# AlexIoannides/bodywork-mlops-demo

Hardware: NVIDIA H100
Metric: train rows/sec (N x 128 least-squares fit) (higher is better)
Workload: dtype bf16x2 (hi+lo) MMA operands, f32 accumulate, f64 fold+solve

## Files before the change

### bodywork-mlops-demo_b200/csrc/b2_api.cu

```cuda
#include <dlfcn.h>
#include <math.h>
#include <stdarg.h>
#include <stdlib.h>

#include <new>
#include <thread>
#include <vector>

#include "b2_internal.cuh"
#include "b2_xchg.cuh"

namespace b2 {

static thread_local char g_err[768] = "";

void set_error(const char* fmt, ...) {
  va_list ap;
  va_start(ap, fmt);
  vsnprintf(g_err, sizeof(g_err), fmt, ap);
  va_end(ap);
}

namespace {

// ... 55 lines not shown
  if (n < 0) { set_error("n_rows < 0"); return B2_E_ARG; }
  if (ldx < d) { set_error("ldx=%lld < d=%d", (long long)ldx, d); return B2_E_ARG; }
  if (mem_kind != B2_MEM_DEVICE && mem_kind != B2_MEM_HOST) { set_error("bad mem_kind %d", mem_kind); return B2_E_ARG; }
  return B2_OK;
}

constexpr int64_t kMaxRowsPerLaunch = (int64_t)1 << 30;

int gram_dispatch(b2_ctx* ctx, const void* X, int x_dtype, const float* y, int64_t n, int d, int64_t ldx,
                  const uint8_t* mask, int keep, bool* tc_last = nullptr, unsigned int* scatter_epoch = nullptr) {
  const int es = x_dtype == B2_F32 ? 4 : 2;
  for (int64_t r0 = 0; r0 < n; r0 += kMaxRowsPerLaunch) {
    const int64_t rows = n - r0 < kMaxRowsPerLaunch ? n - r0 : kMaxRowsPerLaunch;
    const char* Xb = static_cast<const char*>(X) + (size_t)r0 * ldx * es;
    const float* yb = y + r0;
    const uint8_t* mb = mask != nullptr ? mask + r0 : nullptr;
    const bool tc_ok = gram_tc_supported(Xb, x_dtype, yb, rows, d, ldx, mb);
    const bool nw_ok = gram_narrow_supported(Xb, x_dtype, yb, rows, d, ldx, mb);
    int mode = ctx->kernel_mode;
    if (mode == B2_KERNEL_TCGEN05 && !tc_ok) {
      set_error("tensor-core path needs d%%4==0 (fp32) / d%%8==0 (bf16), 16-byte aligned X/y/mask/row pitch, n>=32");
      return B2_E_UNSUPPORTED;
    }
    if (mode == B2_KERNEL_NARROW && !nw_ok) {
      set_error("narrow path needs d<=16, contiguous rows (ldx==d) and 16-byte aligned X/y/mask");
      return B2_E_UNSUPPORTED;
    }
    if (mode == B2_KERNEL_AUTO) {
      if (nw_ok && rows >= 4096) mode = B2_KERNEL_NARROW;
      else mode = (tc_ok && rows >= 2048) ? B2_KERNEL_TCGEN05 : B2_KERNEL_SIMT;
    }
    const int64_t main_rows = mode == B2_KERNEL_NARROW ? gram_narrow_main_rows(rows, d)
                            : mode == B2_KERNEL_TCGEN05 ? gram_tc_main_rows(rows, d, ldx, nullptr) : 0;
    if (main_rows > 0)
      if (int r = launch_gram_shift(ctx, Xb, x_dtype, yb, rows, d, ldx)) return r;
    if (main_rows < rows) {
      if (int r = launch_gram_simt(ctx, Xb + (size_t)main_rows * ldx * es, x_dtype, yb + main_rows, rows - main_rows, d,
                                   ldx, mb != nullptr ? mb + main_rows : nullptr, keep, ctx->s_zero_pending))
        return r;
      ctx->s_zero_pending = false;
    }
    const bool last = r0 + rows == n;
    if (main_rows > 0 && mode == B2_KERNEL_NARROW) {
      if (int r = launch_gram_narrow(ctx, Xb, x_dtype, yb, rows, d, mb, keep, ctx->s_zero_pending)) return r;
      ctx->s_zero_pending = false;
    } else if (main_rows > 0) {
      const unsigned int epoch =
          last && scatter_epoch != nullptr && ctx->n_ranks > 1 && ctx->p2p_ready ? ++ctx->xchg_epoch : 0u;
      if (int r = launch_gram_tc(ctx, Xb, x_dtype, yb, rows, d, ldx, mb, keep, ctx->s_zero_pending, epoch)) return r;
      ctx->s_zero_pending = false;
      if (scatter_epoch != nullptr) *scatter_epoch = epoch;
    }
    if (last && tc_last != nullptr) *tc_last = mode == B2_KERNEL_TCGEN05;
  }
  return B2_OK;
}

int ensure_staging(b2_ctx* ctx) {
  if (ctx->stage_x[0] != nullptr) return B2_OK;
  ctx->stage_rows = 1 << 18;
  ctx->stage_bytes_x = (size_t)ctx->stage_rows * kMaxD * 4;
  for (int b = 0; b < 2; ++b) {
    B2_CUDA(cudaMalloc(&ctx->stage_x[b], ctx->stage_bytes_x));
    B2_CUDA(cudaMalloc(reinterpret_cast<void**>(&ctx->stage_y[b]), (size_t)ctx->stage_rows * 4));
    B2_CUDA(cudaMalloc(reinterpret_cast<void**>(&ctx->stage_m[b]), (size_t)ctx->stage_rows));
    B2_CUDA(cudaEventCreateWithFlags(&ctx->ev_copied[b], cudaEventDisableTiming));
// ... 1596 lines not shown
```

### bodywork-mlops-demo_b200/csrc/b2_internal.cuh

```cuda
#pragma once
#include <cuda.h>
#include <cuda_bf16.h>
#include <cuda_runtime.h>
#include <stdint.h>
#include <stdio.h>
#include <string.h>

#include <type_traits>

#include "../../include/b2gram.h"

namespace b2 {

constexpr int kMaxD = B2_MAX_D;
constexpr int kMaxS = kMaxD + 2;
constexpr int kKernelEventPairs = 64;
constexpr int kMaxRanks = 8;
constexpr size_t kXchgSlotDoubles = (size_t)kMaxS * kMaxS;
constexpr size_t kXchgDataDoubles = 2 * kMaxRanks * kXchgSlotDoubles;
constexpr size_t kXchgBytes = kXchgDataDoubles * sizeof(double) + 256;

constexpr int kTcRows = 64;
constexpr int kTcM = 128;
constexpr int kTcEMax = 16;
// ... 76 lines not shown
  do {                                                                                     \
    cudaError_t e_ = (call);                                                               \
    if (e_ != cudaSuccess) {                                                               \
      b2::set_error("%s failed: %s (%s:%d)", #call, cudaGetErrorString(e_), __FILE__, __LINE__); \
      return B2_E_CUDA;                                                                    \
    }                                                                                      \
  } while (0)

}

struct b2_ctx {
  int device = 0;
  int sm_count = 0;
  size_t hbm_bytes = 0;
  char name[128] = {0};
  cudaStream_t stream = nullptr;
  cudaStream_t copy_stream = nullptr;
  cudaEvent_t ev_t0 = nullptr, ev_t1 = nullptr;
  cudaEvent_t ev_k[b2::kKernelEventPairs][2];
  int k_pairs = 0;
  int64_t launches = 0;

  int kernel_mode = B2_KERNEL_AUTO;
  int drain_rows = 8192;
  int precision = B2_PRECISION_SPLIT;

  int d = 0;
  double* S = nullptr;

  double* tc_part = nullptr;
  double* tc_red = nullptr;
  float* shift = nullptr;
  bool solve_attr_set = false;
  double* solve_host = nullptr;
  struct TmCache {
    const void* X = nullptr; const float* y = nullptr; const uint8_t* mask = nullptr;
    int64_t n = 0, ldx = 0; int d = 0, x_dtype = -1;
    int y_map_2d = 0, m_map_2d = 0;
    alignas(64) unsigned char tmX[128], tmY[128], tmM[128];
  } tm_cache;
  double* simt_part = nullptr;
  int simt_ctas = 0;
  double* score_part = nullptr;
  int score_ctas = 0;
  double* coef_dev = nullptr;
  double* grad_part = nullptr;
  double* refine = nullptr;
  double* loo = nullptr;
  double* loo_part = nullptr;
  double* cv_stage[2] = {nullptr, nullptr};
  int cv_stage_alphas = 0;
  double* enet = nullptr;
  size_t enet_doubles = 0;
  double* folds = nullptr;
  size_t folds_doubles = 0;
  int n_folds = 0;
  int folds_d = 0;
  unsigned long long* fold_range = nullptr;
  double* coef_host = nullptr;
  cudaEvent_t ev_coef[2] = {nullptr, nullptr};
  int coef_slot = 0;
  long long* synth_count = nullptr;
  double* solve_out = nullptr;
  void* stage_x[2] = {nullptr, nullptr};
  float* stage_y[2] = {nullptr, nullptr};
  uint8_t* stage_m[2] = {nullptr, nullptr};
// ... 101 lines not shown
```

### bodywork-mlops-demo_b200/csrc/b2_ptx.cuh

```cuda
#pragma once
#include <cuda_bf16.h>
#include <stdint.h>

namespace b2 {

__device__ __forceinline__ uint32_t smem_u32(const void* p) {
  return static_cast<uint32_t>(__cvta_generic_to_shared(p));
}
__device__ __forceinline__ void mbar_init(uint32_t bar, uint32_t count) {
  asm volatile("mbarrier.init.shared::cta.b64 [%0], %1;" ::"r"(bar), "r"(count));
}
__device__ __forceinline__ void mbar_arrive(uint32_t bar) {
  asm volatile("mbarrier.arrive.shared::cta.b64 _, [%0];" ::"r"(bar) : "memory");
}
__device__ __forceinline__ void mbar_expect_tx(uint32_t bar, uint32_t bytes) {
  asm volatile("mbarrier.arrive.expect_tx.shared::cta.b64 _, [%0], %1;" ::"r"(bar), "r"(bytes) : "memory");
}
__device__ __forceinline__ uint64_t globaltimer_ns() {
  uint64_t t;
  asm volatile("mov.u64 %0, %globaltimer;" : "=l"(t));
  return t;
}
__device__ __forceinline__ void mbar_wait(uint32_t bar, uint32_t parity, uint32_t hint_ns = 20000u) {
  uint32_t done = 0;
  uint64_t t0 = 0;
  while (true) {
    asm volatile(
        "{\n\t.reg .pred p;\n\t"
        "mbarrier.try_wait.parity.shared::cta.b64 p, [%1], %2, %3;\n\t"
        "selp.u32 %0, 1, 0, p;\n\t}"
        : "=r"(done)
        : "r"(bar), "r"(parity), "r"(hint_ns)
        : "memory");
    if (done) break;
    const uint64_t now = globaltimer_ns();
    if (t0 == 0) t0 = now;
    else if (now - t0 > 4000000000ull) __trap();
  }
}
__device__ __forceinline__ void fence_proxy_async_smem() {
  asm volatile("fence.proxy.async.shared::cta;" ::: "memory");
}

__device__ __forceinline__ float ld_shared_f32(uint32_t addr) {
  float v;
  asm volatile("ld.shared.f32 %0, [%1];" : "=f"(v) : "r"(addr));
  return v;
}
__device__ __forceinline__ uint32_t ld_shared_u8(uint32_t addr) {
  uint32_t v;
  asm volatile("ld.shared.u8 %0, [%1];" : "=r"(v) : "r"(addr));
  return v;
}
template <typename T>
__device__ __forceinline__ float raw_ld_shared(uint32_t addr);
template <>
__device__ __forceinline__ float raw_ld_shared<float>(uint32_t addr) { return ld_shared_f32(addr); }
template <>
__device__ __forceinline__ float raw_ld_shared<__nv_bfloat16>(uint32_t addr) {
  unsigned short h;
  asm volatile("ld.shared.u16 %0, [%1];" : "=h"(h) : "r"(addr));
  return __uint_as_float(((uint32_t)h) << 16);
}
template <typename T>
__device__ __forceinline__ float raw_ld_global(const T* p);
template <>
__device__ __forceinline__ float raw_ld_global<float>(const float* p) { return __ldg(p); }
template <>
__device__ __forceinline__ float raw_ld_global<__nv_bfloat16>(const __nv_bfloat16* p) {
  return __bfloat162float(*p);
}
// ... 113 lines not shown
```

### bodywork-mlops-demo_b200/csrc/gram_shift.cu

```cuda
#include <cuda_bf16.h>

#include "b2_internal.cuh"
#include "b2_ptx.cuh"

namespace b2 {
namespace {

constexpr int kShiftBlocks = 64;
constexpr int kShiftStride = kMaxD + 1;
constexpr int kShiftPartOff = kMaxD + 1;
constexpr int kShiftTicketOff = kShiftPartOff + kShiftBlocks * kShiftStride;

__host__ __device__ __forceinline__ int64_t shift_samples(int64_t n) { return n < 2048 ? n : 2048; }

__device__ __forceinline__ float shift_round(float c, bool round_bf16) {
  return round_bf16 ? __bfloat162float(__float2bfloat16_rn(c)) : c;
}
__device__ __noinline__ float shift_value(const float* sp, int j, bool round_bf16) {
  float acc = 0.f;
  int cnt = 0;
#pragma unroll 8
  for (int b = 0; b < kShiftBlocks; ++b) {
    const float p = sp[b * kShiftStride + j];
    if (p == p) { acc += p; ++cnt; }
  }
  return shift_round(cnt > 0 ? acc / (float)cnt : 0.f, round_bf16);
}

constexpr int kShiftCols = 160;
constexpr int kShiftGroups = 4;

template <typename T>
__global__ void __launch_bounds__(kShiftCols * kShiftGroups)
tc_shift_kernel(const T* __restrict__ X, const float* __restrict__ y, int64_t n, int d, int64_t ldx, float* shift) {
  __shared__ float sub[kShiftGroups][kShiftCols];
  __shared__ int subn[kShiftGroups][kShiftCols];
  __shared__ bool last_block;
  __shared__ float part_s[kShiftBlocks * kShiftStride];
  float* sp = shift + kShiftPartOff;
  const int j = threadIdx.x % kShiftCols, g = threadIdx.x / kShiftCols;
  const int64_t samples = shift_samples(n);
  const int64_t stride = n / samples;
  const int64_t per = (samples + kShiftBlocks - 1) / kShiftBlocks;
  const int64_t s0 = blockIdx.x * per;
  const int64_t s1 = (s0 + per < samples) ? s0 + per : samples;
  float acc = 0.f;
  int cnt = 0;
  if (j <= d) {
#pragma unroll 8
    for (int64_t s = s0 + g; s < s1; s += kShiftGroups) {
      const int64_t row = s * stride;
      const float v = (j < d) ? raw_ld_global<T>(X + row * ldx + j) : __ldg(y + row);
      const bool finite = fabsf(v) <= 3.0e38f;
      acc += finite ? v : 0.f;
      cnt += finite ? 1 : 0;
    }
  }
  sub[g][j] = acc;
  subn[g][j] = cnt;
  __syncthreads();
  if (g == 0 && j <= d) {
    const int c = subn[0][j] + subn[1][j] + subn[2][j] + subn[3][j];
    sp[blockIdx.x * kShiftStride + (j == d ? kMaxD : j)] =
        c > 0 ? (((sub[0][j] + sub[1][j]) + sub[2][j]) + sub[3][j]) / (float)c : __int_as_float(0x7fc00000);
    __threadfence();
  }
  __syncthreads();
  unsigned int* ticket = reinterpret_cast<unsigned int*>(shift + kShiftTicketOff);
  if (threadIdx.x == 0) last_block = atomicAdd(ticket, 1u) == gridDim.x - 1;
  __syncthreads();
  if (!last_block) return;
// ... 33 lines not shown
```

### bodywork-mlops-demo_b200/csrc/gram_tc.cu

```cuda
#include <cuda_bf16.h>
#include <stdlib.h>

#include "b2_internal.cuh"
#include "b2_ptx.cuh"
#include "b2_shift.cuh"
#include "b2_xchg.cuh"

namespace b2 {
namespace {

constexpr int kConsumerWGs = 2;
constexpr int kXformWarps = 8;
constexpr int kThreads = 128 * (kConsumerWGs + 2);
constexpr int kFirstXformWarp = 4 * kConsumerWGs;
constexpr int kTmaWarp = kFirstXformWarp;
constexpr int kEWarp = kFirstXformWarp + 1;
static_assert(kFirstXformWarp + kXformWarps == kThreads / 32, "warp roles");
constexpr int kProducers = kXformWarps;
constexpr int kConsumerWarps = 4 * kConsumerWGs;
constexpr int kKGroups = kTcRows / 8;
constexpr uint32_t kRawStageBytes = kTcRows * kMaxD * 4;
constexpr uint32_t kOpSBO = 128;
constexpr uint32_t kOpLBO = (16 + 2 + 16) * kOpSBO;
constexpr uint32_t kOpEOff = 16 * kOpSBO;
// ... 295 lines not shown
  uint8_t* smem = smem_raw + (sbase - smem_u32(smem_raw));
  const int warp = threadIdx.x >> 5;
  const int lane = threadIdx.x & 31;

  const uint32_t bar_raw_full = sbase + G::kOffBar;
  const uint32_t bar_raw_empty = bar_raw_full + 8 * kRawStages;
  const uint32_t bar_op_full = bar_raw_empty + 8 * kRawStages;
  const uint32_t bar_op_empty = bar_op_full + 8 * kOpStages;
  float* shift_s = reinterpret_cast<float*>(smem + G::kOffShift);

  const int64_t total_tiles = (n_rows + kTcRows - 1) / kTcRows;
  const int64_t tile_begin = (int64_t)blockIdx.x * total_tiles / gridDim.x;
  const int64_t tile_end = (int64_t)(blockIdx.x + 1) * total_tiles / gridDim.x;
  const int my_tiles = (int)(tile_end - tile_begin);

  if (threadIdx.x == 0) {
    for (int s = 0; s < kRawStages; ++s) {
      mbar_init(bar_raw_full + 8 * s, 1);
      mbar_init(bar_raw_empty + 8 * s, kProducers + (RAWB ? kConsumerWarps : 0));
    }
    for (int s = 0; s < kOpStages; ++s) {
      mbar_init(bar_op_full + 8 * s, kProducers);
      mbar_init(bar_op_empty + 8 * s, kConsumerWarps);
    }
    asm volatile("fence.mbarrier_init.release.cluster;" ::: "memory");
  }
  if (warp == kTmaWarp && lane == 0) {
    tma_prefetch_desc(&tmX);
    tma_prefetch_desc(&tmY);
    if (has_mask) tma_prefetch_desc(&tmM);
  }
  for (uint32_t o = threadIdx.x * 16; o < kOpStages * kOpStageBytes; o += kThreads * 16)
    *reinterpret_cast<uint4*>(smem + kOffOp + o) = make_uint4(0, 0, 0, 0);
  for (int j = threadIdx.x; j <= kMaxD; j += kThreads)
    shift_s[j] = j == kMaxD ? shift[kMaxD] : (j < pack * d_orig ? shift[j % d_orig] : 0.f);
  fence_proxy_async_smem();
  __syncthreads();

  if (warp < kConsumerWarps) {
    asm volatile("setmaxnreg.inc.sync.aligned.u32 %0;" ::"n"(G::kConsumerRegs));
    auto consume = [&](auto wg_c) {
      constexpr int WG = decltype(wg_c)::value;
      constexpr int kF1 = kTcM - 64 * WG;
      constexpr int kF2 = RAWB ? kF1 : kTcM;
      constexpr int kC1 = 64 * WG;
      constexpr int kR1 = (kF1 + EW) / 2, kR2 = (kF2 + EW) / 2;
      float acc1[kR1], acc2[kR2];
      double* my_part = part + (size_t)blockIdx.x * kTcAccElems;
      auto store = [&](auto n_regs, int dst_acc, int col0, bool add, auto val) {
        const int ln = (int)lane_id(), row0 = 64 * WG + 16 * (warp & 3) + (ln >> 2);
#pragma unroll
        for (int r = 0; r < decltype(n_regs)::value; ++r) {
          const int col = col0 + 8 * (r >> 2) + 2 * (ln & 3) + (r & 1), h = (r >> 1) & 1, i = row0 + 8 * h;
          const bool lower = dst_acc == 0 && col < kTcM && i > col;
          put_f64(my_part + tc_part_index(dst_acc, i, col, EW), val(r, col, h), add, !lower);
        }
      };
      auto drain = [&](const auto& acc, int dst_acc, int col0, bool add) {
        constexpr int kR = sizeof(acc) / sizeof(float);
        if constexpr (RAWB) {
          constexpr int kF = 2 * kR - EW;
          const double s1[2] = {(double)__shfl_sync(0xffffffffu, acc[kF / 2], lane & ~3),
                                (double)__shfl_sync(0xffffffffu, acc[kF / 2 + 2], lane & ~3)};
          store(std::integral_constant<int, kR>{}, dst_acc, col0, add, [&](int r, int col, int h) {
            return col < kTcM ? (double)acc[r] - (double)shift_s[col] * s1[h] : (double)acc[r];
          });
// ... 38 lines not shown
        wgmma_commit();
        const bool last = (in_chunk == chunk_tiles - 1) || (it == my_tiles - 1);
        if (last) {
          wgmma_wait<0>();
          fence_regs(acc1);
          if constexpr (SPLIT) fence_regs(acc2);
        } else {
          wgmma_wait<1>();
        }
        if (lane == 0) {
          if (held >= 0) release(held);
          if (last) release(it);
        }
        held = last ? -1 : it;
        if (last) {
          drain(acc1, 0, kC1, !first_chunk);
          first_chunk = false;
          in_chunk = 0;
        } else {
          ++in_chunk;
        }
        if (++os == kOpStages) { os = 0; oph ^= 1; }
      }
      wgmma_wait<0>();
      if constexpr (SPLIT) {
        fence_regs(acc2);
        drain(acc2, RAWB ? 0 : 1, RAWB ? kC1 : 0, RAWB);
      }
    };
    if (__shfl_sync(0xffffffffu, warp, 0) >= 4) consume(std::integral_constant<int, 1>{});
    else consume(std::integral_constant<int, 0>{});
  } else {
    asm volatile("setmaxnreg.dec.sync.aligned.u32 %0;" ::"n"(G::kProducerRegs));
    const uint32_t tx = (uint32_t)(kTcRows * d * sizeof(T)) + kTcRows * pack * 4 + (has_mask ? kTcRows * pack : 0);
    auto issue = [&](int j) {
      const int s = j % kRawStages;
      mbar_wait(bar_raw_empty + 8 * s, ((uint32_t)(j / kRawStages) & 1u) ^ 1u, wait_ns);
      const uint32_t full = bar_raw_full + 8 * s;
      mbar_expect_tx(full, tx);
      const int64_t row0 = (tile_begin + j) * kTcRows;
      tma_load_2d(sbase + kOffRaw + s * kRawStageBytes, &tmX, 0, (int)row0, full);
      if constexpr (RAWB) tma_load_2d(sbase + kOffRaw + s * kRawStageBytes + kRawBoxBytes, &tmX, 64, (int)row0, full);
      const int sub0 = (int)row0 * pack;
      if (y_map_2d) tma_load_2d(sbase + kOffY + s * kYStageBytes, &tmY, 0, sub0 >> 2, full);
      else tma_load_1d(sbase + kOffY + s * kYStageBytes, &tmY, sub0, full);
      if (has_mask == 2) tma_load_2d(sbase + kOffMask + s * kMStageBytes, &tmM, 0, sub0 >> 4, full);
      else if (has_mask) tma_load_1d(sbase + kOffMask + s * kMStageBytes, &tmM, sub0, full);
    };
    const bool issuer = warp == kTmaWarp && lane == 0;
    if (issuer)
      for (int j = 0; j < G::kAhead && j < my_tiles; ++j) issue(j);

    const int t = warp - kFirstXformWarp;
    const int nb = (d + 63) >> 6;
    const int i = 64 * (t % nb) + 2 * lane;
    const uint32_t swp = ((uint32_t)lane >> 2) & 1u;
    const uint32_t st_off = (uint32_t)((i >> 3) * kOpSBO + (i & 7) * 16);
    auto esum = [&]() { return sbase + G::kOffESum + 8 * lane_id(); };
    if (warp == kEWarp) { st_shared_f64(esum(), 0.0); st_shared_f64(esum() + 256, 0.0); st_shared_f64(esum() + 512, 0.0); }
    int rs = 0, os = 0;
    uint32_t rph = 0, oph = 0;
    for (int it = 0; it < my_tiles; ++it) {
      if (issuer && it + G::kAhead < my_tiles) issue(it + G::kAhead);
      __syncwarp();
      mbar_wait(bar_raw_full + 8 * rs, rph, wait_ns);
      mbar_wait(bar_op_empty + 8 * os, oph ^ 1, wait_ns);
      const int64_t row0 = (tile_begin + it) * kTcRows;
      const int64_t left = n_rows - row0;
      const int rows_valid = left < kTcRows ? (int)left : kTcRows;
      const bool full_tile = (!has_mask) && (rows_valid == kTcRows);
      const uint32_t raw_addr = sbase + kOffRaw + rs * kRawStageBytes;
      const uint32_t m_addr = sbase + kOffMask + rs * kMStageBytes;
      const uint32_t op_addr = sbase + kOffOp + os * kOpStageBytes;
      if (warp == kEWarp && !(dbg & 192u)) {
        const uint32_t y_addr = sbase + kOffY + rs * kYStageBytes;
        const uint32_t e_addr = op_addr + kOpEOff;
        const float c_y = shift_s[kMaxD];
        float a = 0.f, b = 0.f, c = 0.f;
        for (int half = 0; half < kTcRows / 32; ++half) {
          const int rr = lane + 32 * half;
          const uint32_t dst = e_addr + (rr >> 3) * kOpLBO + (rr & 7) * 2;
          for (int bl = 0; bl < pack; ++bl) {
            const int sub = rr * pack + bl;
            bool use = rr < rows_valid;
            if (use && has_mask) use = (ld_shared_u8(m_addr + sub) == (uint32_t)keep);
// ... 87 lines not shown
    }
    if (warp == kEWarp) {
      const uint32_t es = esum();
      double sy = ld_shared_f64(es), syy = ld_shared_f64(es + 256), cnt = ld_shared_f64(es + 512);
#pragma unroll
      for (int o = 16; o > 0; o >>= 1) {
        sy += __shfl_xor_sync(0xffffffffu, sy, o);
        syy += __shfl_xor_sync(0xffffffffu, syy, o);
        cnt += __shfl_xor_sync(0xffffffffu, cnt, o);
      }
      if (lane == 0) {
        double* ys = part + (size_t)gridDim.x * kTcAccElems + kTcSums * blockIdx.x;
        ys[0] = sy; ys[1] = syy; ys[2] = cnt;
      }
    }
  }
}

struct TcFinal {
  int assign;
  int n_ranks, rank;
  unsigned int epoch;
  PeerPtrs peers;
};

constexpr int kFinalizeThreads = 1024;
constexpr int kFinalizeCtas = (kRedElems + kFinalizeThreads / 4 - 1) / (kFinalizeThreads / 4);

__global__ void __launch_bounds__(kFinalizeThreads, 1)
tc_finalize_kernel(const double* part, int n_ctas, double* red, const float* __restrict__ shift, int d, int pack,
                   int ew, int d2, double* S, unsigned int* sync, const TcFinal fin) {
  __shared__ double quarter[kFinalizeThreads];
  __shared__ double c_s[kMaxD + 1];
  for (int j = threadIdx.x; j <= kMaxD; j += blockDim.x) c_s[j] = (double)shift[j];
  {
    constexpr int epb = kFinalizeThreads / 4;
    const int n_acc = tc_part_elems(ew, d2 != 0);
    const int n_red = n_acc + kTcSums;
    const int per = (((n_red + (int)gridDim.x - 1) / (int)gridDim.x) + epb - 1) / epb * epb;
    const int e0 = (int)blockIdx.x * per;
    const int e1 = e0 + per < n_red ? e0 + per : n_red;
    if (e0 < n_red) tc_reduce_range(part, n_ctas, n_acc, red, e0, e1, quarter);
  }
  grid_barrier(sync + 0);
  {
    const int dp = d + 2;
    const int total = dp * dp;
    const size_t slot = xchg_slot_offset(fin.epoch, fin.rank);
    for (int idx = (int)(blockIdx.x * blockDim.x + threadIdx.x); idx < total; idx += (int)(gridDim.x * blockDim.x)) {
      const double val = tc_fold_value(red, c_s, d, pack, ew, d2 != 0, idx);
      const double sv = fin.assign ? val : S[idx] + val;
      S[idx] = sv;
      if (fin.n_ranks > 1) xchg_store_all(fin.peers, fin.n_ranks, slot, idx, sv);
    }
    if (fin.n_ranks > 1) __threadfence_system();
  }
  __syncthreads();
  __shared__ bool last_cta;
  if (threadIdx.x == 0) {
    __threadfence();
    last_cta = (atomicAdd(sync + 2, 1u) == gridDim.x - 1);
    if (last_cta) {
      sync[0] = 0u; sync[2] = 0u;
      __threadfence();
    }
  }
// ... 62 lines not shown
  CUtensorMap& tmX = *tmX_out;
  memset(tmM_out, 0, sizeof(*tmM_out));
  *m_map_2d_out = 0;
  {
    cuuint64_t dims[2] = {(cuuint64_t)d, (cuuint64_t)n};
    cuuint64_t strides[1] = {(cuuint64_t)ldx * es};
    cuuint32_t box[2] = {(cuuint32_t)(swz64 ? 64 : d_box), (cuuint32_t)kTcRows};
    cuuint32_t estr[2] = {1, 1};
    CUresult r = encode(&tmX, x_dtype == B2_F32 ? CU_TENSOR_MAP_DATA_TYPE_FLOAT32 : CU_TENSOR_MAP_DATA_TYPE_BFLOAT16,
                        2, const_cast<void*>(X), dims, strides, box, estr, CU_TENSOR_MAP_INTERLEAVE_NONE,
                        swz64 ? CU_TENSOR_MAP_SWIZZLE_128B : CU_TENSOR_MAP_SWIZZLE_NONE, CU_TENSOR_MAP_L2_PROMOTION_L2_256B,
                        CU_TENSOR_MAP_FLOAT_OOB_FILL_NONE);
    if (r != CUDA_SUCCESS) {
      set_error("cuTensorMapEncodeTiled(X) failed with %d (n=%lld d=%d box=%d ldx=%lld)", (int)r, (long long)n, d, d_box,
                (long long)ldx);
      return B2_E_CUDA;
    }
  }
  if (int r = encode_vec(encode, tmY_out, CU_TENSOR_MAP_DATA_TYPE_FLOAT32, 4, y, n_y, y_box, y_map_2d_out, "y")) return r;
  if (mask == nullptr) return B2_OK;
  return encode_vec(encode, tmM_out, CU_TENSOR_MAP_DATA_TYPE_UINT8, 1, mask, n_y, y_box, m_map_2d_out, "mask");
}

int64_t gram_tc_main_rows(int64_t n_in, int d_in, int64_t ldx_in, int* pack_out) {
  int pack = 1;
  if (d_in > 16 && d_in <= 64 && ldx_in == d_in) {
    pack = 128 / d_in;
    if (pack > kMaxPack) pack = kMaxPack;
    if (n_in < (int64_t)2 * kTcRows * pack) pack = 1;
  }
  const int group = pack == 1 ? 1 : (pack == 3 ? 48 : (pack == 5 ? 80 : 16));
  if (pack_out != nullptr) *pack_out = pack;
  return n_in - n_in % group;
}

int launch_gram_tc(b2_ctx* ctx, const void* X, int x_dtype, const float* y, int64_t n_in, int d_in, int64_t ldx_in,
                   const uint8_t* mask, int keep, bool assign, unsigned int scatter_epoch) {
  PFN_encodeTiled encode = get_encode();
  if (encode == nullptr) {
    set_error("cuTensorMapEncodeTiled is not available from the driver");
    return B2_E_CUDA;
  }
  const int es = x_dtype == B2_F32 ? 4 : 2;
  int pack = 1;
  const int64_t n_main = gram_tc_main_rows(n_in, d_in, ldx_in, &pack);
  const int64_t n = n_main / pack;
  const int d = pack > 1 ? 128 : d_in;
  const int d_tensor = d_in * pack;
  const int64_t ldx = ldx_in * pack;
  const int64_t n_y = n_main;
  const bool rawb = x_dtype == B2_BF16 && d_in == 128 && pack == 1;
  CUtensorMap tmX, tmY, tmM;
  b2_ctx::TmCache& tc = ctx->tm_cache;
  const bool cached = tc.X == X && tc.y == y && tc.mask == mask && tc.n == n_in && tc.ldx == ldx_in && tc.d == d_in &&
                      tc.x_dtype == x_dtype;
  if (cached) {
    memcpy(&tmX, tc.tmX, sizeof(tmX)); memcpy(&tmY, tc.tmY, sizeof(tmY)); memcpy(&tmM, tc.tmM, sizeof(tmM));
  } else {
    int y_map_2d = 0, m_map_2d = 0;
    if (int r = encode_maps(encode, X, x_dtype, es, y, n, d_tensor, d, ldx, n_y, pack, mask, rawb, &tmX, &tmY, &tmM, &y_map_2d,
                            &m_map_2d))
      return r;
    tc.X = X; tc.y = y; tc.mask = mask; tc.n = n_in; tc.ldx = ldx_in; tc.d = d_in; tc.x_dtype = x_dtype;
    tc.y_map_2d = y_map_2d; tc.m_map_2d = m_map_2d;
    memcpy(tc.tmX, &tmX, sizeof(tmX)); memcpy(tc.tmY, &tmY, sizeof(tmY)); memcpy(tc.tmM, &tmM, sizeof(tmM));
  }
// ... 11 lines not shown
  }();
#else
  constexpr uint32_t wait_ns = 20000u;
#endif
#ifdef B2_DEV_KNOBS
  static const uint32_t dbg = []() {
    const char* e = getenv("B2_TC_DEBUG");
    return e ? (uint32_t)atoi(e) : 0u;
  }();
#else
  constexpr uint32_t dbg = 0u;
#endif
  const bool split = ctx->precision == B2_PRECISION_SPLIT;
  const int ew = tc_e_width(pack);
  const bool d2 = split && !rawb;
  decltype(&gram_tc_kernel<float, 0, false>) kernel = nullptr;
  uint32_t smem = TcGeo<false>::kSmemBytes;
  with_rows(x_dtype, X, [&](auto* Xr) {
    using T = row_t<decltype(Xr)>;
    return with_int<0, 1>(split, [&](auto SP) {
      constexpr bool kSplit = decltype(SP)::value;
      if (d != 128) kernel = gram_tc_kernel<T, 0, kSplit>;
      else if (ew == 16) kernel = gram_tc_kernel<T, 128, kSplit, false, 16>;
      else kernel = gram_tc_kernel<T, 128, kSplit>;
      if constexpr (std::is_same_v<T, __nv_bfloat16>) {
        if (rawb) {
          kernel = gram_tc_kernel<T, 128, kSplit, true>;
          smem = TcGeo<true>::kSmemBytes;
        }
      }
      return B2_OK;
    });
  });
  B2_CUDA(cudaFuncSetAttribute(kernel, cudaFuncAttributeMaxDynamicSharedMemorySize, smem));
  const int pair = ctx->k_pairs % kKernelEventPairs;
  B2_CUDA(cudaEventRecord(ctx->ev_k[pair][0], ctx->stream));
  kernel<<<grid, kThreads, smem, ctx->stream>>>(tmX, tmY, tmM, tc.y_map_2d, mask != nullptr ? 1 + tc.m_map_2d : 0, keep,
                                                n, d, pack, d_in, ctx->shift, chunk_tiles, ctx->tc_part, wait_ns, dbg);
  B2_CUDA(cudaGetLastError());
  B2_CUDA(cudaEventRecord(ctx->ev_k[pair][1], ctx->stream));
  ctx->k_pairs += 1;

  TcFinal fin;
  memset(&fin, 0, sizeof(fin));
  fin.assign = assign ? 1 : 0;
  fin.n_ranks = 1;
  if (scatter_epoch != 0) {
    fin.n_ranks = ctx->n_ranks; fin.rank = ctx->rank; fin.epoch = scatter_epoch;
    for (int r = 0; r < kMaxRanks; ++r) fin.peers.p[r] = ctx->xchg_peer[r];
  }
  {
    cudaLaunchConfig_t cfg;
    memset(&cfg, 0, sizeof(cfg));
    cfg.gridDim = dim3(kFinalizeCtas < sms ? kFinalizeCtas : sms);
    cfg.blockDim = dim3(kFinalizeThreads); cfg.dynamicSmemBytes = 0; cfg.stream = ctx->stream;
    cudaLaunchAttribute attr[1];
    attr[0].id = cudaLaunchAttributeCooperative;
    attr[0].val.cooperative = 1;
    cfg.attrs = attr; cfg.numAttrs = 1;
    const double* part_arg = ctx->tc_part;
    const float* shift_arg = ctx->shift;
    B2_CUDA(cudaLaunchKernelEx(&cfg, tc_finalize_kernel, part_arg, grid, ctx->tc_red, shift_arg, d_in, pack, ew,
                               d2 ? 1 : 0, ctx->S, ctx->tc_sync, fin));
  }
  ctx->launches += 2;
  return B2_OK;
}

}
```

### bodywork-mlops-demo_b200/csrc/solve.cu

```cuda
#include "b2_internal.cuh"
#include "b2_xchg.cuh"

namespace b2 {
namespace {

constexpr int kOutIntercept = kMaxD;
constexpr int kOutInfo = kMaxD + 1;
constexpr int kOutRank = kMaxD + 2;
constexpr int kOutSingular = kMaxD + 3;
constexpr int kOutRows = kOutSingular + kMaxD;

struct LdcgStat {
  const double* S;
  __device__ __forceinline__ double operator()(int i) const { return __ldcg(S + i); }
};

template <class Stat>
__device__ void build_normal_equations_of(const Stat& S, int d, double alpha, int fit_intercept,
                                       double* A, double* r, double* mean, double* ybar_out) {
  const int dp = d + 2, pitch = d + 1;
  const double n = S(d * dp + d);
  const double inv_n = n > 0.0 ? 1.0 / n : 0.0;
  double sxy = 0.0;
  if ((int)threadIdx.x < d) {
    const double sx = S(threadIdx.x * dp + d);
    sxy = S(threadIdx.x * dp + d + 1);
    mean[threadIdx.x] = fit_intercept ? sx * inv_n : 0.0;
  }
  const double ybar = fit_intercept ? S(d * dp + d + 1) * inv_n : 0.0;
  __syncthreads();
  if ((int)threadIdx.x < d) r[threadIdx.x] = sxy - n * mean[threadIdx.x] * ybar;
  const int lane = threadIdx.x & 31, warp = threadIdx.x >> 5, nwarps = blockDim.x >> 5;
  for (int i0 = warp; i0 < d; i0 += 2 * nwarps) {
// ... 32 lines not shown
  const double t = fma(er, er, er);
  return fma(y, t, y);
}

struct SolveXchg {
  double* own;
  int n_ranks;
  unsigned int epoch;
  unsigned long long timeout_ns;
};

constexpr int kNB = 16;
constexpr int kCholThreads = 512;
constexpr int kUPitch = kNB + 1;

__device__ void refine_update(const double* S, int d, int fit_intercept, bool singular, const double* dbeta, double* misc,
                              double* __restrict__ rf, double* __restrict__ out);

template <bool REFINE>
__global__ void __launch_bounds__(kCholThreads, 1)
solve_cholesky_kernel(double* S, int d, double alpha, int fit_intercept, double* __restrict__ out, const SolveXchg xc,
                      double* __restrict__ rf) {
  extern __shared__ double sm[];
  const int pitch = d + 1;
  double* A = sm;
  double* r = A + d * pitch;
  double* mean = A + (d + 1) * pitch;
  double* invd = mean + d;
  double* misc = invd + d;
  double* U = misc + 8;
  const int tid = threadIdx.x, lane = tid & 31;
  const int warp = __shfl_sync(0xffffffffu, tid >> 5, 0);
  long long tm[5] = {0, 0, 0, 0, 0};
  long long tc0 = clock64();
  if (xc.own != nullptr) {
    __shared__ int ok;
    if (tid == 0) ok = xchg_wait(xc.own, xc.n_ranks, xc.epoch, xc.timeout_ns) ? 1 : 0;
    __syncthreads();
    if (!ok) {
      if (tid == 0) {
        xchg_flags(xc.own)[kXchgStatusWord] = xc.epoch;
        out[kOutInfo] = -1.0;
      }
      return;
    }
    const int dp = d + 2;
    for (int base = 0; base < dp * dp; base += 4 * blockDim.x) {
      double sv[4];
#pragma unroll
      for (int u = 0; u < 4; ++u) {
        const int idx = base + u * blockDim.x + tid;
        sv[u] = idx < dp * dp ? xchg_sum(xc.own, xc.n_ranks, xc.epoch, idx) : 0.0;
      }
#pragma unroll
      for (int u = 0; u < 4; ++u) {
        const int idx = base + u * blockDim.x + tid;
        if (idx < dp * dp) S[idx] = sv[u];
      }
    }
    __threadfence();
    __syncthreads();
  }
  build_normal_equations(S, d, alpha, fit_intercept, A, r, mean, &misc[0]);
  if constexpr (REFINE) {
    if (tid < d) r[tid] = rf[kRfGrad + tid] - alpha * rf[kRfBeta + tid];
    __syncthreads();
// ... 1408 lines not shown
  const size_t chol = (size_t)(d + 1) * (d + 1) + 3 * d + 16 + (size_t)(d + 1) * kUPitch;
  const size_t eig = (size_t)(d + 1) * (d + 1) + 3 * d + 16 + 4 * kMaxD + kMaxD + 2 * (kMaxD + 8) + kMaxD;
  return sizeof(double) * (chol > eig ? chol : eig);
}

int ensure_solve_attrs(b2_ctx* ctx) {
  if (!ctx->solve_attr_set) {
    const int bytes = (int)solve_smem_bytes(kMaxD);
    B2_CUDA(cudaFuncSetAttribute(solve_cholesky_kernel<false>, cudaFuncAttributeMaxDynamicSharedMemorySize, bytes));
    B2_CUDA(cudaFuncSetAttribute(solve_cholesky_kernel<true>, cudaFuncAttributeMaxDynamicSharedMemorySize, bytes));
    B2_CUDA(cudaFuncSetAttribute(solve_spectral_kernel, cudaFuncAttributeMaxDynamicSharedMemorySize, bytes));
    B2_CUDA(cudaFuncSetAttribute(solve_eigvals_kernel, cudaFuncAttributeMaxDynamicSharedMemorySize, bytes));
    B2_CUDA(cudaFuncSetAttribute(solve_eigh_kernel, cudaFuncAttributeMaxDynamicSharedMemorySize,
                                 (int)eigh_smem_bytes(kMaxD)));
    B2_CUDA(cudaFuncSetAttribute(solve_enet_kernel, cudaFuncAttributeMaxDynamicSharedMemorySize,
                                 (int)enet_smem_bytes(kMaxD)));
    B2_CUDA(cudaFuncSetAttribute(bayes_ridge_kernel, cudaFuncAttributeMaxDynamicSharedMemorySize,
                                 (int)bayes_smem_bytes(kMaxD)));
    B2_CUDA(cudaFuncSetAttribute(ard_kernel, cudaFuncAttributeMaxDynamicSharedMemorySize, (int)ard_smem_bytes(kMaxD)));
    ctx->solve_attr_set = true;
  }
  return B2_OK;
}

}

int launch_solve_cholesky(b2_ctx* ctx, double alpha, int fit_intercept, unsigned int gather_epoch) {
  if (int r = ensure_solve_attrs(ctx)) return r;
  SolveXchg xc;
  xc.own = gather_epoch != 0 ? ctx->xchg : nullptr;
  xc.n_ranks = ctx->n_ranks;
  xc.epoch = gather_epoch;
  xc.timeout_ns = ctx->xchg_timeout_ns;
  solve_cholesky_kernel<false><<<1, kCholThreads, solve_smem_bytes(ctx->d), ctx->stream>>>(ctx->S, ctx->d, alpha,
                                                                                           fit_intercept, ctx->solve_host,
                                                                                           xc, nullptr);
  B2_CUDA(cudaGetLastError());
  ctx->launches += 1;
  return B2_OK;
}

int launch_solve_refine(b2_ctx* ctx, double alpha, int fit_intercept) {
  if (int r = ensure_solve_attrs(ctx)) return r;
  SolveXchg xc;
  xc.own = nullptr;
  xc.n_ranks = 1;
  xc.epoch = 0;
  xc.timeout_ns = 0;
  solve_cholesky_kernel<true><<<1, kCholThreads, solve_smem_bytes(ctx->d), ctx->stream>>>(ctx->S, ctx->d, alpha,
                                                                                          fit_intercept, ctx->solve_host,
                                                                                          xc, ctx->refine);
  B2_CUDA(cudaGetLastError());
  ctx->launches += 1;
  return B2_OK;
}

int launch_solve_spectral(b2_ctx* ctx, double cond, int fit_intercept) {
  if (int r = ensure_solve_attrs(ctx)) return r;
  solve_spectral_kernel<<<1, 512, solve_smem_bytes(ctx->d), ctx->stream>>>(ctx->S, ctx->d, cond, fit_intercept, ctx->solve_out);
  B2_CUDA(cudaGetLastError());
  ctx->launches += 1;
  return B2_OK;
}

int launch_solve_eigh(b2_ctx* ctx, int fit_intercept) {
  if (int r = ensure_solve_attrs(ctx)) return r;
  solve_eigh_kernel<<<1, kEighThreads, eigh_smem_bytes(ctx->d), ctx->stream>>>(ctx->S, ctx->d, fit_intercept, ctx->loo);
  B2_CUDA(cudaGetLastError());
  ctx->launches += 1;
  return B2_OK;
// ... 38 lines not shown
```

Measured before the change: 5.369 billion.

## Use programmatic dependent launch to overlap gram TC prologue with shift kernel

Launches the tensor-core gram kernel and the Cholesky solve kernel with programmatic stream serialization. Predecessor kernels signal launch_dependents early, and the gram kernel now issues its first TMA loads before griddepcontrol.wait so its prologue overlaps the tail of the shift kernel. The per-launch cudaFuncSetAttribute calls are also cached once per context. The risk is that X/y loads issued before the wait do not depend on shift, so this is only correct if the shift kernel does not write those buffers. The start timing event now also covers the shift kernel.

```diff
diff --git a/bodywork-mlops-demo_b200/csrc/b2_api.cu b/bodywork-mlops-demo_b200/csrc/b2_api.cu
--- a/bodywork-mlops-demo_b200/csrc/b2_api.cu
+++ b/bodywork-mlops-demo_b200/csrc/b2_api.cu
@@ -111,6 +111,8 @@
     }
     const int64_t main_rows = mode == B2_KERNEL_NARROW ? gram_narrow_main_rows(rows, d)
                             : mode == B2_KERNEL_TCGEN05 ? gram_tc_main_rows(rows, d, ldx, nullptr) : 0;
+    if (main_rows > 0 && mode == B2_KERNEL_TCGEN05)
+      B2_CUDA(cudaEventRecord(ctx->ev_k[ctx->k_pairs % kKernelEventPairs][0], ctx->stream));
     if (main_rows > 0)
       if (int r = launch_gram_shift(ctx, Xb, x_dtype, yb, rows, d, ldx)) return r;
     if (main_rows < rows) {
diff --git a/bodywork-mlops-demo_b200/csrc/b2_internal.cuh b/bodywork-mlops-demo_b200/csrc/b2_internal.cuh
--- a/bodywork-mlops-demo_b200/csrc/b2_internal.cuh
+++ b/bodywork-mlops-demo_b200/csrc/b2_internal.cuh
@@ -132,6 +132,7 @@
   double* tc_red = nullptr;
   float* shift = nullptr;
   bool solve_attr_set = false;
+  bool gram_attr_set = false;
   double* solve_host = nullptr;
   struct TmCache {
     const void* X = nullptr; const float* y = nullptr; const uint8_t* mask = nullptr;
diff --git a/bodywork-mlops-demo_b200/csrc/b2_ptx.cuh b/bodywork-mlops-demo_b200/csrc/b2_ptx.cuh
--- a/bodywork-mlops-demo_b200/csrc/b2_ptx.cuh
+++ b/bodywork-mlops-demo_b200/csrc/b2_ptx.cuh
@@ -37,6 +37,10 @@
     if (t0 == 0) t0 = now;
     else if (now - t0 > 4000000000ull) __trap();
   }
+}
+__device__ __forceinline__ void grid_dep_wait() { asm volatile("griddepcontrol.wait;" ::: "memory"); }
+__device__ __forceinline__ void grid_dep_launch_dependents() {
+  asm volatile("griddepcontrol.launch_dependents;" ::: "memory");
 }
 __device__ __forceinline__ void fence_proxy_async_smem() {
   asm volatile("fence.proxy.async.shared::cta;" ::: "memory");
diff --git a/bodywork-mlops-demo_b200/csrc/gram_shift.cu b/bodywork-mlops-demo_b200/csrc/gram_shift.cu
--- a/bodywork-mlops-demo_b200/csrc/gram_shift.cu
+++ b/bodywork-mlops-demo_b200/csrc/gram_shift.cu
@@ -37,6 +37,7 @@
   __shared__ int subn[kShiftGroups][kShiftCols];
   __shared__ bool last_block;
   __shared__ float part_s[kShiftBlocks * kShiftStride];
+  grid_dep_launch_dependents();
   float* sp = shift + kShiftPartOff;
   const int j = threadIdx.x % kShiftCols, g = threadIdx.x / kShiftCols;
   const int64_t samples = shift_samples(n);
diff --git a/bodywork-mlops-demo_b200/csrc/gram_tc.cu b/bodywork-mlops-demo_b200/csrc/gram_tc.cu
--- a/bodywork-mlops-demo_b200/csrc/gram_tc.cu
+++ b/bodywork-mlops-demo_b200/csrc/gram_tc.cu
@@ -351,6 +351,26 @@
   }
   for (uint32_t o = threadIdx.x * 16; o < kOpStages * kOpStageBytes; o += kThreads * 16)
     *reinterpret_cast<uint4*>(smem + kOffOp + o) = make_uint4(0, 0, 0, 0);
+  const uint32_t tx = (uint32_t)(kTcRows * d * sizeof(T)) + kTcRows * pack * 4 + (has_mask ? kTcRows * pack : 0);
+  auto issue = [&](int j) {
+    const int s = j % kRawStages;
+    mbar_wait(bar_raw_empty + 8 * s, ((uint32_t)(j / kRawStages) & 1u) ^ 1u, wait_ns);
+    const uint32_t full = bar_raw_full + 8 * s;
+    mbar_expect_tx(full, tx);
+    const int64_t row0 = (tile_begin + j) * kTcRows;
+    tma_load_2d(sbase + kOffRaw + s * kRawStageBytes, &tmX, 0, (int)row0, full);
+    if constexpr (RAWB) tma_load_2d(sbase + kOffRaw + s * kRawStageBytes + kRawBoxBytes, &tmX, 64, (int)row0, full);
+    const int sub0 = (int)row0 * pack;
+    if (y_map_2d) tma_load_2d(sbase + kOffY + s * kYStageBytes, &tmY, 0, sub0 >> 2, full);
+    else tma_load_1d(sbase + kOffY + s * kYStageBytes, &tmY, sub0, full);
+    if (has_mask == 2) tma_load_2d(sbase + kOffMask + s * kMStageBytes, &tmM, 0, sub0 >> 4, full);
+    else if (has_mask) tma_load_1d(sbase + kOffMask + s * kMStageBytes, &tmM, sub0, full);
+  };
+  const bool issuer = warp == kTmaWarp && lane == 0;
+  __syncthreads();
+  if (issuer)
+    for (int j = 0; j < G::kAhead && j < my_tiles; ++j) issue(j);
+  grid_dep_wait();
   for (int j = threadIdx.x; j <= kMaxD; j += kThreads)
     shift_s[j] = j == kMaxD ? shift[kMaxD] : (j < pack * d_orig ? shift[j % d_orig] : 0.f);
   fence_proxy_async_smem();
@@ -455,25 +475,6 @@
     else consume(std::integral_constant<int, 0>{});
   } else {
     asm volatile("setmaxnreg.dec.sync.aligned.u32 %0;" ::"n"(G::kProducerRegs));
-    const uint32_t tx = (uint32_t)(kTcRows * d * sizeof(T)) + kTcRows * pack * 4 + (has_mask ? kTcRows * pack : 0);
-    auto issue = [&](int j) {
-      const int s = j % kRawStages;
-      mbar_wait(bar_raw_empty + 8 * s, ((uint32_t)(j / kRawStages) & 1u) ^ 1u, wait_ns);
-      const uint32_t full = bar_raw_full + 8 * s;
-      mbar_expect_tx(full, tx);
-      const int64_t row0 = (tile_begin + j) * kTcRows;
-      tma_load_2d(sbase + kOffRaw + s * kRawStageBytes, &tmX, 0, (int)row0, full);
-      if constexpr (RAWB) tma_load_2d(sbase + kOffRaw + s * kRawStageBytes + kRawBoxBytes, &tmX, 64, (int)row0, full);
-      const int sub0 = (int)row0 * pack;
-      if (y_map_2d) tma_load_2d(sbase + kOffY + s * kYStageBytes, &tmY, 0, sub0 >> 2, full);
-      else tma_load_1d(sbase + kOffY + s * kYStageBytes, &tmY, sub0, full);
-      if (has_mask == 2) tma_load_2d(sbase + kOffMask + s * kMStageBytes, &tmM, 0, sub0 >> 4, full);
-      else if (has_mask) tma_load_1d(sbase + kOffMask + s * kMStageBytes, &tmM, sub0, full);
-    };
-    const bool issuer = warp == kTmaWarp && lane == 0;
-    if (issuer)
-      for (int j = 0; j < G::kAhead && j < my_tiles; ++j) issue(j);
-
     const int t = warp - kFirstXformWarp;
     const int nb = (d + 63) >> 6;
     const int i = 64 * (t % nb) + 2 * lane;
@@ -627,6 +628,7 @@
                    int ew, int d2, double* S, unsigned int* sync, const TcFinal fin) {
   __shared__ double quarter[kFinalizeThreads];
   __shared__ double c_s[kMaxD + 1];
+  grid_dep_launch_dependents();
   for (int j = threadIdx.x; j <= kMaxD; j += blockDim.x) c_s[j] = (double)shift[j];
   {
     constexpr int epb = kFinalizeThreads / 4;
@@ -755,6 +757,28 @@
   const int group = pack == 1 ? 1 : (pack == 3 ? 48 : (pack == 5 ? 80 : 16));
   if (pack_out != nullptr) *pack_out = pack;
   return n_in - n_in % group;
+}
+
+static int ensure_gram_tc_attrs(b2_ctx* ctx) {
+  if (ctx->gram_attr_set) return B2_OK;
+  const auto attr = cudaFuncAttributeMaxDynamicSharedMemorySize;
+  const int smem = (int)TcGeo<false>::kSmemBytes, smem_rawb = (int)TcGeo<true>::kSmemBytes;
+  B2_CUDA(cudaFuncSetAttribute(gram_tc_kernel<float, 0, false>, attr, smem));
+  B2_CUDA(cudaFuncSetAttribute(gram_tc_kernel<float, 0, true>, attr, smem));
+  B2_CUDA(cudaFuncSetAttribute(gram_tc_kernel<float, 128, false>, attr, smem));
+  B2_CUDA(cudaFuncSetAttribute(gram_tc_kernel<float, 128, true>, attr, smem));
+  B2_CUDA(cudaFuncSetAttribute(gram_tc_kernel<float, 128, false, false, 16>, attr, smem));
+  B2_CUDA(cudaFuncSetAttribute(gram_tc_kernel<float, 128, true, false, 16>, attr, smem));
+  B2_CUDA(cudaFuncSetAttribute(gram_tc_kernel<__nv_bfloat16, 0, false>, attr, smem));
+  B2_CUDA(cudaFuncSetAttribute(gram_tc_kernel<__nv_bfloat16, 0, true>, attr, smem));
+  B2_CUDA(cudaFuncSetAttribute(gram_tc_kernel<__nv_bfloat16, 128, false>, attr, smem));
+  B2_CUDA(cudaFuncSetAttribute(gram_tc_kernel<__nv_bfloat16, 128, true>, attr, smem));
+  B2_CUDA(cudaFuncSetAttribute(gram_tc_kernel<__nv_bfloat16, 128, false, false, 16>, attr, smem));
+  B2_CUDA(cudaFuncSetAttribute(gram_tc_kernel<__nv_bfloat16, 128, true, false, 16>, attr, smem));
+  B2_CUDA(cudaFuncSetAttribute(gram_tc_kernel<__nv_bfloat16, 128, false, true>, attr, smem_rawb));
+  B2_CUDA(cudaFuncSetAttribute(gram_tc_kernel<__nv_bfloat16, 128, true, true>, attr, smem_rawb));
+  ctx->gram_attr_set = true;
+  return B2_OK;
 }
 
 int launch_gram_tc(b2_ctx* ctx, const void* X, int x_dtype, const float* y, int64_t n_in, int d_in, int64_t ldx_in,
@@ -832,13 +856,21 @@
       return B2_OK;
     });
   });
-  B2_CUDA(cudaFuncSetAttribute(kernel, cudaFuncAttributeMaxDynamicSharedMemorySize, smem));
-  const int pair = ctx->k_pairs % kKernelEventPairs;
-  B2_CUDA(cudaEventRecord(ctx->ev_k[pair][0], ctx->stream));
-  kernel<<<grid, kThreads, smem, ctx->stream>>>(tmX, tmY, tmM, tc.y_map_2d, mask != nullptr ? 1 + tc.m_map_2d : 0, keep,
-                                                n, d, pack, d_in, ctx->shift, chunk_tiles, ctx->tc_part, wait_ns, dbg);
-  B2_CUDA(cudaGetLastError());
-  B2_CUDA(cudaEventRecord(ctx->ev_k[pair][1], ctx->stream));
+  if (int r = ensure_gram_tc_attrs(ctx)) return r;
+  {
+    cudaLaunchConfig_t cfg;
+    memset(&cfg, 0, sizeof(cfg));
+    cfg.gridDim = dim3(grid); cfg.blockDim = dim3(kThreads); cfg.dynamicSmemBytes = smem; cfg.stream = ctx->stream;
+    cudaLaunchAttribute attr[1];
+    attr[0].id = cudaLaunchAttributeProgrammaticStreamSerialization;
+    attr[0].val.programmaticStreamSerializationAllowed = 1;
+    cfg.attrs = attr; cfg.numAttrs = 1;
+    const int has_mask = mask != nullptr ? 1 + tc.m_map_2d : 0;
+    const float* shift_arg = ctx->shift;
+    B2_CUDA(cudaLaunchKernelEx(&cfg, kernel, tmX, tmY, tmM, tc.y_map_2d, has_mask, keep, n, d, pack, d_in, shift_arg,
+                               chunk_tiles, ctx->tc_part, wait_ns, dbg));
+  }
+  B2_CUDA(cudaEventRecord(ctx->ev_k[ctx->k_pairs % kKernelEventPairs][1], ctx->stream));
   ctx->k_pairs += 1;
 
   TcFinal fin;
diff --git a/bodywork-mlops-demo_b200/csrc/solve.cu b/bodywork-mlops-demo_b200/csrc/solve.cu
--- a/bodywork-mlops-demo_b200/csrc/solve.cu
+++ b/bodywork-mlops-demo_b200/csrc/solve.cu
@@ -1,4 +1,5 @@
 #include "b2_internal.cuh"
+#include "b2_ptx.cuh"
 #include "b2_xchg.cuh"
 
 namespace b2 {
@@ -97,6 +98,7 @@
   const int tid = threadIdx.x, lane = tid & 31;
   const int warp = __shfl_sync(0xffffffffu, tid >> 5, 0);
   long long tm[5] = {0, 0, 0, 0, 0};
+  grid_dep_wait();
   long long tc0 = clock64();
   if (xc.own != nullptr) {
     __shared__ int ok;
@@ -1571,10 +1573,17 @@
   xc.n_ranks = ctx->n_ranks;
   xc.epoch = gather_epoch;
   xc.timeout_ns = ctx->xchg_timeout_ns;
-  solve_cholesky_kernel<false><<<1, kCholThreads, solve_smem_bytes(ctx->d), ctx->stream>>>(ctx->S, ctx->d, alpha,
-                                                                                           fit_intercept, ctx->solve_host,
-                                                                                           xc, nullptr);
-  B2_CUDA(cudaGetLastError());
+  cudaLaunchConfig_t cfg;
+  memset(&cfg, 0, sizeof(cfg));
+  cfg.gridDim = dim3(1); cfg.blockDim = dim3(kCholThreads);
+  cfg.dynamicSmemBytes = solve_smem_bytes(ctx->d); cfg.stream = ctx->stream;
+  cudaLaunchAttribute attr[1];
+  attr[0].id = cudaLaunchAttributeProgrammaticStreamSerialization;
+  attr[0].val.programmaticStreamSerializationAllowed = 1;
+  cfg.attrs = attr; cfg.numAttrs = 1;
+  double* no_refine = nullptr;
+  B2_CUDA(cudaLaunchKernelEx(&cfg, solve_cholesky_kernel<false>, ctx->S, ctx->d, alpha, fit_intercept, ctx->solve_host,
+                             xc, no_refine));
   ctx->launches += 1;
   return B2_OK;
 }
```

After: 5.343 billion, median of 6. No clear change (-0.5%).
